# ponimatkin/freepose

Hardware: AMD Instinct MI355X
Metric: proposals/sec (ViT-L feat + top-k + 576-pose render-compare) (higher is better)
Workload: dtype bf16

## Files before the change

freepose_amd/_lib.py:

```python
from __future__ import annotations

import ctypes as C
import os
from pathlib import Path

_HERE = Path(__file__).resolve().parent
LIB_PATH = _HERE / "lib" / "libfreepose_hip.so"
LAB_LIB_PATH = _HERE / "lib" / "libfreepose_hip_lab.so"

_lib = None
_use_lab = False


def use_lab():
    global _use_lab
    if _lib is not None and not _use_lab:
        raise RuntimeError("use_lab() after the product library was loaded")
    _use_lab = True


def is_lab() -> bool:
    return _use_lab

c_void_p, c_int, c_float, c_double, c_size_t, c_char_p = C.c_void_p, C.c_int, C.c_float, C.c_double, C.c_size_t, C.c_char_p
P = C.POINTER


class VitArch(C.Structure):
    _fields_ = [("dim", c_int), ("depth", c_int), ("heads", c_int), ("mlp_dim", c_int), ("patch", c_int),
                ("n_reg", c_int), ("pos_grid", c_int), ("ln_eps", c_float)]


class ClipArch(C.Structure):
    _fields_ = [("width", c_int), ("depth", c_int), ("heads", c_int), ("mlp_dim", c_int), ("patch", c_int), ("grid", c_int),
                ("embed_dim", c_int), ("ln_eps", c_float), ("quick_gelu", c_int)]


class ClipTextArch(C.Structure):
    _fields_ = [("width", c_int), ("depth", c_int), ("heads", c_int), ("mlp_dim", c_int), ("vocab", c_int), ("ctx", c_int),
                ("embed_dim", c_int), ("ln_eps", c_float)]


SIGNATURES = {
    "fp_last_error": (c_char_p, []),
    "fp_version": (c_int, []),
    "fp_ctx_create": (c_int, [c_int, P(c_void_p)]),
    "fp_ctx_destroy": (c_int, [c_void_p]),
    "fp_ctx_set_option": (c_int, [c_void_p, c_char_p, c_int]),
    "fp_ctx_workspace_bytes": (c_size_t, [c_void_p]),
    "fp_vit_create": (c_int, [c_void_p, P(VitArch), P(c_void_p)]),
    "fp_vit_destroy": (c_int, [c_void_p]),
    "fp_vit_set_weight": (c_int, [c_void_p, c_char_p, c_void_p, c_size_t, c_void_p]),
    "fp_vit_forward": (c_int, [c_void_p, c_void_p, c_int, c_int, c_int, c_int, c_int, c_void_p, c_void_p]),
    "fp_vit_flops": (c_double, [c_void_p, c_int, c_int, c_int, c_int]),
    "fp_ffa": (c_int, [c_void_p, c_void_p, c_void_p, c_int, c_int, c_int, c_int, c_int, c_int, c_void_p, c_void_p, c_void_p]),
    "fp_bank_prepare": (c_int, [c_void_p, c_void_p, c_int, c_int, c_void_p, c_void_p]),
    "fp_bank_topk": (c_int, [c_void_p, c_void_p, c_int, c_int, c_void_p, c_int, c_int, c_int, c_void_p, c_void_p, c_void_p]),
    "fp_topk_merge": (c_int, [c_void_p, c_void_p, c_void_p, c_int, c_int, c_int, c_void_p, c_void_p, c_void_p]),
    "fp_rerank_views": (c_int, [c_void_p, c_void_p, c_void_p, c_void_p, c_void_p, c_int, c_int, c_int, c_int, c_void_p, c_void_p]),
    "fp_l2_normalize": (c_int, [c_void_p, c_void_p, c_int, c_int, c_void_p, c_void_p]),
    "fp_template_score": (c_int, [c_void_p, c_void_p, c_void_p, c_void_p, c_int, c_int, c_int, c_void_p, c_void_p]),
    "fp_template_score_normed": (c_int, [c_void_p, c_void_p, c_void_p, c_void_p, c_int, c_int, c_int, c_void_p, c_void_p]),
    "fp_crop_resize_pad": (c_int, [c_void_p, c_void_p, c_int, c_int, c_int, c_int, c_int, c_void_p, c_int, c_float,
                                   c_int, c_void_p, c_int, c_void_p, c_int, c_void_p]),
    "fp_roi_align": (c_int, [c_void_p, c_void_p, c_int, c_int, c_int, c_int, c_void_p, c_int, c_int, c_int, c_int, c_float,
                             c_void_p, c_void_p]),
    "fp_generate_rotations": (c_int, [c_int, c_void_p]),
    "fp_geodesic_select": (c_int, [c_void_p, c_void_p, c_int, c_void_p, c_double, c_void_p, P(c_int), c_void_p]),
    "fp_mesh_upload": (c_int, [c_void_p, c_void_p, c_int, c_void_p, c_int, c_void_p, P(c_void_p)]),
    "fp_mesh_upload_textured": (c_int, [c_void_p, c_void_p, c_int, c_void_p, c_int, c_void_p, c_void_p, c_int, c_int, c_void_p,
                                        P(c_void_p)]),
    "fp_mesh_set_ambient": (c_int, [c_void_p, c_float]),
    "fp_mesh_set_shading": (c_int, [c_void_p, c_int]),
    "fp_mesh_set_filter": (c_int, [c_void_p, c_int]),
    "fp_mesh_set_cull": (c_int, [c_void_p, c_int]),
    "fp_project_vertices": (c_int, [c_void_p, c_void_p, c_void_p, c_int, c_float, c_float, c_float, c_float, c_float, c_void_p,
                                    c_void_p, c_void_p]),
    "fp_mesh_destroy": (c_int, [c_void_p]),
    "fp_rasterize": (c_int, [c_void_p, c_void_p, c_void_p, c_int, c_float, c_float, c_float, c_float, c_float, c_int,
                             c_int, c_void_p, c_void_p, c_void_p]),
    "fp_rasterize_extents": (c_int, [c_void_p, c_void_p, c_void_p, c_int, c_float, c_float, c_float, c_float, c_float, c_int,
                                     c_int, c_void_p, c_void_p, c_void_p, c_void_p, c_void_p]),
    "fp_depth_extents": (c_int, [c_void_p, c_void_p, c_int, c_int, c_int, c_float, c_float, c_float, c_float, c_void_p,
                                 c_void_p]),
    "fp_chamfer": (c_int, [c_void_p, c_void_p, c_int, c_void_p, c_void_p, c_int, c_int, c_int, c_int, c_void_p, c_void_p]),
    "fp_depth_compare": (c_int, [c_void_p, c_void_p, c_void_p, c_int, c_int, c_int, c_void_p, c_int, c_void_p, c_void_p, c_void_p, c_int,
# ... 117 lines not shown
```

freepose_amd/csrc/clip.hip:

```cpp
#include "../../include/freepose_hip.h"
#include "tower_steps.h"

namespace {

constexpr float CLIP_MEAN[3] = {0.48145466f, 0.4578275f, 0.40821073f}, CLIP_SD[3] = {0.26862954f, 0.26130258f, 0.27577711f};

}

struct fp_clip {
    fp_ctx* ctx = nullptr;
    fp_clip_arch a{};
    TowerEmbedW emb;
    const bf16_t *lnprew = nullptr, *lnpreb = nullptr, *lnpostw = nullptr, *lnpostb = nullptr;
    bool have_conv = false;
    ClipTowerCommon tw;
};

extern "C" int fp_clip_create(fp_ctx* ctx, const fp_clip_arch* arch, fp_clip** out) {
    FP_REQUIRE(ctx && arch && out, "clip_create: null argument");
    FP_REQUIRE(arch->quick_gelu == 0, "clip_create: quick_gelu towers are not provided (exact-erf GELU only)");
    if (int rc = ClipTowerCommon::check_arch("clip_create", arch->width, arch->heads, arch->mlp_dim, arch->embed_dim, arch->depth,
                                             arch->patch > 0 && arch->grid > 0, "patch, grid")) return rc;
    fp_clip* v = new fp_clip();
    v->ctx = ctx;
// ... 48 lines not shown
    fp_set_error("clip_set_weight: unknown tensor name '%s'", name);
    return FP_ERR_INVALID;
}

extern "C" int fp_clip_encode_image(fp_clip* v, const void* d_images, int B, int S, void* d_out, void* stream) {
    FP_REQUIRE(v && d_images && d_out, "clip_encode_image: null argument");
    const fp_clip_arch& a = v->a;
    hipStream_t s = (hipStream_t)stream;
    FP_REQUIRE(B > 0, "clip_encode_image: B=%d", B);
    FP_REQUIRE(S == a.patch * a.grid, "clip_encode_image: images are %d x %d, the tower takes %d x %d (patch %d, grid %d: the positional "
               "embedding is not interpolated)", S, S, a.patch * a.grid, a.patch * a.grid, a.patch, a.grid);
    FP_REQUIRE(v->have_conv && v->tw.have_proj && v->emb.cls && v->emb.pos && v->lnprew && v->lnpreb && v->lnpostw && v->lnpostb,
               "clip_encode_image: embedding / ln_pre / ln_post / proj weights not set");
    int rc;
    if ((rc = v->tw.all_blocks_complete("clip_encode_image"))) return rc;
    const int D = a.width, P = a.grid * a.grid, n_tok = P + 1;
    const int npad = cdiv(n_tok, 16) * 16;
    const size_t M = (size_t)B * npad;
    if ((rc = fp_tower_offsets_fit("clip_encode_image", M, D, a.mlp_dim, B))) return rc;

    bf16_t *A0, *X, *Y, *QKV, *AO, *H1, *POOL;
    fp_ctx* ctx = v->ctx;
    FP_WS(ctx, "clip.im2col", (size_t)B * P * v->emb.KP * 2, A0);
    FP_WS(ctx, "clip.x", M * D * 2, X);
    FP_WS(ctx, "clip.y", M * D * 2, Y);
    FP_WS(ctx, "clip.qkv", M * 3 * D * 2, QKV);
    FP_WS(ctx, "clip.ao", M * D * 2, AO);
    FP_WS(ctx, "clip.h1", M * (size_t)a.mlp_dim * 2, H1);
    FP_WS(ctx, "clip.pool", (size_t)B * D * 2, POOL);

    bf16_t* R = Y;
    bf16_t* T = X;
    const TowerRun t{ctx, nullptr, s, B, n_tok, npad, D, a.mlp_dim, a.ln_eps, R, T, AO, H1, v->tw.ones};
    if ((rc = fp_tower_embed(t, v->emb, v->emb.pos + D, (const bf16_t*)d_images, S, S, A0, X))) return rc;
    if ((rc = fp_layernorm(X, Y, v->lnprew, v->lnpreb, (int)M, D, a.ln_eps, 0, 0, 0, s))) return rc;
    if ((rc = fp_tower_blocks(t, v->tw.blk, QKV, a.heads, v->tw.head_dim, false))) return rc;
    if ((rc = fp_layernorm(R, POOL, v->lnpostw, v->lnpostb, B, D, a.ln_eps, 1, npad, 0, s))) return rc;
    return v->tw.project(ctx, POOL, D, a.embed_dim, d_out, B, s);
}

extern "C" double fp_clip_flops(const fp_clip* v, int B) {
    if (!v) return 0.0;
    const fp_clip_arch& a = v->a;
    const double P = (double)a.grid * a.grid, N = P + 1, D = a.width, Mm = a.mlp_dim;
    const double per_block = 8.0 * N * D * D + 4.0 * N * D * Mm + 4.0 * N * N * D;
    return B * (a.depth * per_block + 2.0 * P * (3.0 * a.patch * a.patch) * D + 2.0 * D * a.embed_dim);
}
```

freepose_amd/csrc/tower_steps.h:

```cpp
#pragma once
#include <stdio.h>
#include <string.h>

#include <cmath>

#include "internal.h"

struct GemmStep {
    FpGemmArgs g{};
    int epi;
    GemmStep(const bf16_t* X, int ldx, const bf16_t* W, int K, bf16_t* C, int ldc, const bf16_t* bias, int M, int N, bool gelu = false)
        : epi(gelu ? FP_EPI_BIAS_GELU : FP_EPI_BIAS) {
        g.X = X; g.ldx = ldx; g.W = W; g.ldw = K; g.C = C; g.ldc = ldc; g.bias = bias;
        g.M = M; g.N = N; g.K = K;
    }
    GemmStep& residual(const bf16_t* gamma, const bf16_t* resid, int ldr, float2* stat_part = nullptr) {
        g.gamma = gamma; g.resid = resid; g.ldr = ldr; g.stat_part = stat_part;
        epi = stat_part ? FP_EPI_LS_RES_STATS : FP_EPI_BIAS_LS_RES;
        return *this;
    }
    GemmStep& transposed_v(int npad, int heads) {
        g.ldc = 8; g.npad = npad; g.heads = heads;
        epi = FP_EPI_VT;
        return *this;
// ... 44 lines not shown
            if (hipEventCreate(&e.a) != hipSuccess || hipEventCreate(&e.b) != hipSuccess) return;
            p->ev_pool.push_back(e);
        }
        slot = p->ev_used++;
        p->ev_pool[slot].cls = cls;
        (void)hipEventRecord(p->ev_pool[slot].a, s);
    }
    ~ProfScope() {
        if (slot != (size_t)-1) (void)hipEventRecord(p->ev_pool[slot].b, s);
    }
};

struct TowerBlockW {
    const bf16_t *n1w = nullptr, *n1b = nullptr, *qkvw = nullptr, *qkvb = nullptr, *projw = nullptr,
                 *projb = nullptr, *ls1 = nullptr, *n2w = nullptr, *n2b = nullptr, *fc1w = nullptr, *fc1b = nullptr,
                 *fc2w = nullptr, *fc2b = nullptr, *ls2 = nullptr;
    bool complete() const { return n1w && n1b && qkvw && qkvb && projw && projb && n2w && n2b && fc1w && fc1b && fc2w && fc2b; }
};
struct TowerRun {
    fp_ctx* ctx; TowerProf* prof; hipStream_t s;
    int B, n_tok, npad, D, mlp_dim;
    float eps;
    bf16_t *R, *T, *AO, *H1;
    const bf16_t* ones;
    int M() const { return B * npad; }
    void count(double flops_per_row, int launches) const { if (prof) prof->count((double)B * n_tok * flops_per_row, launches); }
};
struct TowerEmbedW {
    int patch = 0, KP = 0, n_reg = 0;
    const float *mean = nullptr, *sd = nullptr;
    bf16_t* pe_w = nullptr;
    const bf16_t *pe_b = nullptr, *cls = nullptr, *pos = nullptr, *reg = nullptr;
};
inline int fp_tower_embed(const TowerRun& t, const TowerEmbedW& e, const bf16_t* pos_patch, const bf16_t* img, int H, int W, bf16_t* A0, bf16_t* X) {
    const int P = (H / e.patch) * (W / e.patch);
    int rc;
    {
        ProfScope ps(t.prof, t.s, TOWER_OTHER);
        if ((rc = fp_im2col_norm_ms(img, A0, t.B, H, W, e.patch, e.KP, e.mean, e.sd, t.s))) return rc;
        if ((rc = fp_token_init(X, e.cls, e.pos, e.reg, e.n_reg, t.B, t.n_tok, t.npad, t.D, t.s))) return rc;
    }
    ProfScope ps(t.prof, t.s, TOWER_GEMM);
    GemmStep pe(A0, e.KP, e.pe_w, e.KP, X, t.D, e.pe_b, t.B * P, t.D);
    if ((rc = pe.patch_embed(pos_patch, P, t.npad, 1 + e.n_reg).run(t.ctx, t.s))) return rc;
    if (t.prof) t.prof->count(2.0 * t.B * P * (3.0 * e.patch * e.patch) * t.D, 1);
    return FP_OK;
}
inline int fp_tower_out_proj(const TowerRun& t, const TowerBlockW& w, float2* stat_part) {
    ProfScope ps(t.prof, t.s, TOWER_GEMM);
    GemmStep proj(t.AO, t.D, w.projw, t.D, t.R, t.D, w.projb, t.M(), t.D);
    if (int rc = proj.residual(w.ls1 ? w.ls1 : t.ones, t.R, t.D, stat_part).run(t.ctx, t.s)) return rc;
    t.count(2.0 * t.D * t.D, 1);
    return FP_OK;
}
inline int fp_tower_mlp(const TowerRun& t, const TowerBlockW& w, LnStats* st, const bf16_t* fc1w, const uint4* fc1_cb, float2* stat_part) {
    const int D = t.D, M = t.M(), N = t.mlp_dim;
    int rc;
    {
        ProfScope ps(t.prof, t.s, TOWER_OTHER);
        if ((rc = st ? st->ready(nullptr, N, t.s) : fp_layernorm(t.R, t.T, w.n2w, w.n2b, M, D, t.eps, 0, 0, 0, t.s))) return rc;
    }
    ProfScope ps(t.prof, t.s, TOWER_GEMM);
    GemmStep fc1(st ? t.R : t.T, D, st ? fc1w : w.fc1w, D, t.H1, N, w.fc1b, M, N, true);
    if (st && (rc = st->attach(fc1, fc1_cb))) return rc;
    if ((rc = fc1.run(t.ctx, t.s))) return rc;
    if ((rc = GemmStep(t.H1, N, w.fc2w, N, t.R, D, w.fc2b, M, D).residual(w.ls2 ? w.ls2 : t.ones, t.R, D, stat_part).run(t.ctx, t.s))) return rc;
    t.count(4.0 * D * N, 2);
    return FP_OK;
}

inline bool fp_weight_numel(const char* who, const char* name, size_t numel, size_t want) {
    if (numel != want) fp_set_error("%s: %s has %zu elements, expected %zu", who, name, numel, want);
// ... 104 lines not shown
```

freepose_amd/csrc/vit.hip:

```cpp
#include <stdio.h>

#include "../../include/freepose_hip.h"
#include "tower_steps.h"

struct fp_vit {
    fp_ctx* ctx = nullptr;
    fp_vit_arch a{};
    TowerEmbedW emb;
    const bf16_t *normw = nullptr, *normb = nullptr;
    bf16_t* ones = nullptr;
    std::vector<TowerBlockW> blk;
    struct VitFold { bf16_t *qkvw = nullptr, *fc1w = nullptr; uint4 *qkv_cb = nullptr, *fc1_cb = nullptr; };
    std::vector<VitFold> fold;
    int folded_upto = 0;
    hipEvent_t fold_ev = nullptr;
    hipStream_t fold_stream = nullptr;
    bool refold = false;
    std::map<std::pair<int, int>, bf16_t*> pos_cache;
    TowerProf prof;
};

extern "C" int fp_vit_create(fp_ctx* ctx, const fp_vit_arch* arch, fp_vit** out) {
    FP_REQUIRE(ctx && arch && out, "vit_create: null argument");
    FP_REQUIRE(arch->dim % 64 == 0 && arch->heads * 64 == arch->dim, "vit_create: dim=%d heads=%d (head dim must be 64)",
// ... 85 lines not shown
        if (rc) { (void)hipFree(buf); return rc; }
        it = v->pos_cache.emplace(key, buf).first;
    }
    *out = it->second;
    return FP_OK;
}

static int vit_fold(fp_vit* v, int first, int L, hipStream_t s) {
    const fp_vit_arch& a = v->a;
    const size_t D = a.dim, Mm = a.mlp_dim;
    for (int i = first; i < L; ++i) {
        const TowerBlockW& w = v->blk[i];
        fp_vit::VitFold& f = v->fold[i];
        if (!f.qkvw) FP_HIP(hipMalloc((void**)&f.qkvw, 3 * D * D * 2));
        if (!f.qkv_cb) FP_HIP(hipMalloc((void**)&f.qkv_cb, 3 * D * sizeof(uint4)));
        if (!f.fc1w) FP_HIP(hipMalloc((void**)&f.fc1w, Mm * D * 2));
        if (!f.fc1_cb) FP_HIP(hipMalloc((void**)&f.fc1_cb, Mm * sizeof(uint4)));
        int rc;
        if ((rc = fp_ln_fold(w.qkvw, w.n1w, w.n1b, w.qkvb, f.qkvw, f.qkv_cb, (int)(3 * D), (int)D, (int)D, FP_ATTN_QSCALE, s))) return rc;
        if ((rc = fp_ln_fold(w.fc1w, w.n2w, w.n2b, w.fc1b, f.fc1w, f.fc1_cb, (int)Mm, (int)D, 0, 1.0f, s))) return rc;
    }
    return FP_OK;
}

extern "C" double fp_vit_flops(const fp_vit* v, int B, int H, int W, int layer) {
    const fp_vit_arch& a = v->a;
    const double P = (double)(H / a.patch) * (W / a.patch), N = P + 1 + a.n_reg, D = a.dim;
    const int L = std::min(layer, a.depth);
    const double mlp_ratio = (double)a.mlp_dim / a.dim;
    const double per_block = (8.0 + 4.0 * mlp_ratio) * N * D * D + 4.0 * N * N * D;
    return B * (L * per_block + 2.0 * P * (3.0 * a.patch * a.patch) * D);
}

extern "C" int fp_vit_forward(fp_vit* v, const void* d_images, int B, int H, int W, int layer, int feature_type,
                              void* d_out, void* stream) {
    FP_REQUIRE(v && d_images && d_out, "vit_forward: null argument");
    const fp_vit_arch& a = v->a;
    hipStream_t s = (hipStream_t)stream;
    fp_ctx* ctx = v->ctx;
    FP_REQUIRE(B > 0 && H % a.patch == 0 && W % a.patch == 0, "vit_forward: B=%d H=%d W=%d (patch %d)", B, H, W, a.patch);
    FP_REQUIRE(feature_type >= 0 && feature_type <= 3, "vit_forward: feature_type %d", feature_type);
    FP_REQUIRE(v->emb.cls && v->emb.pos && v->emb.pe_b && v->normw && v->normb && (a.n_reg == 0 || v->emb.reg),
               "vit_forward: embedding / final-norm weights not set");
    const int L = (layer >= 1 && layer <= a.depth) ? layer : a.depth;
    for (int i = 0; i < L; ++i) {
        FP_REQUIRE(v->blk[i].complete(), "vit_forward: weights of block %d not set", i);
    }
    const int D = a.dim, gh = H / a.patch, gw = W / a.patch, P = gh * gw;
    const int n_tok = P + 1 + a.n_reg;
    const int npad = cdiv(n_tok, 16) * 16;
    const size_t M = (size_t)B * npad;
    FP_REQUIRE(M * (size_t)a.mlp_dim * 2 < 0xffffffffull, "vit_forward: batch too large for 32-bit tile offsets (B=%d)", B);
    const int Mi = (int)M;

    bf16_t *A0, *X, *Y, *QK, *Vt, *AO, *H1;
    int rc;
    const bool lnf = ctx->opt_ln_fused != 0 && D % 64 == 0;
    LnStats st{nullptr, nullptr, nullptr, Mi, D, a.ln_eps};
    if (lnf) {
        if (v->fold_ev && s != v->fold_stream) FP_HIP(hipStreamWaitEvent(s, v->fold_ev, 0));
        if (v->folded_upto < L) {
            if (v->refold) {
                FP_HIP(hipDeviceSynchronize());
                v->refold = false;
            }
            if ((rc = vit_fold(v, v->folded_upto, L, s))) return rc;
            if (!v->fold_ev) FP_HIP(hipEventCreateWithFlags(&v->fold_ev, hipEventDisableTiming));
            FP_HIP(hipEventRecord(v->fold_ev, s));
            v->fold_stream = s;
            v->folded_upto = L;
        }
        FP_WS(ctx, "vit.ln_stat", M * sizeof(uint4), st.stat);
        FP_WS(ctx, "vit.ln_rstd", M * sizeof(float), st.rstd);
        FP_WS(ctx, "vit.ln_part", M * (size_t)(D / 64) * sizeof(float2), st.part);
    }
    FP_WS(ctx, "vit.im2col", (size_t)B * P * v->emb.KP * 2, A0);
    FP_WS(ctx, "vit.x", M * D * 2, X);
    FP_WS(ctx, "vit.y", M * D * 2, Y);
    FP_WS(ctx, "vit.qk", M * 2 * D * 2, QK);
    FP_WS(ctx, "vit.vt", M * D * 2 + 256, Vt);
    FP_WS(ctx, "vit.ao", M * D * 2, AO);
    FP_WS(ctx, "vit.h1", M * (size_t)a.mlp_dim * 2, H1);

    const bf16_t* pos_patch;
    if ((rc = vit_pos(v, gh, gw, s, &pos_patch))) return rc;

    const TowerRun t{ctx, &v->prof, s, B, n_tok, npad, D, a.mlp_dim, a.ln_eps, X, Y, AO, H1, v->ones};
    if ((rc = fp_tower_embed(t, v->emb, pos_patch, (const bf16_t*)d_images, H, W, A0, X))) return rc;
    const bf16_t* in = lnf ? X : Y;
    for (int i = 0; i < L; ++i) {
        const TowerBlockW& w = v->blk[i];
        const fp_vit::VitFold& f = v->fold[i];
        {
            ProfScope ps(&v->prof, s, TOWER_OTHER);
            if ((rc = lnf ? st.ready(i == 0 ? X : nullptr, 2 * D, s) : fp_layernorm(X, Y, w.n1w, w.n1b, Mi, D, a.ln_eps, 0, 0, 0, s))) return rc;
        }
        {
            ProfScope ps(&v->prof, s, TOWER_GEMM);
            const bf16_t* qkvw = lnf ? f.qkvw : w.qkvw;
            GemmStep qk(in, D, qkvw, D, QK, 2 * D, w.qkvb, Mi, 2 * D), vt(in, D, qkvw + (size_t)2 * D * D, D, Vt, 8, w.qkvb + 2 * D, Mi, D);
            vt.transposed_v(npad, a.heads);
            if (lnf && ((rc = st.attach(qk, f.qkv_cb)) || (rc = st.attach(vt, f.qkv_cb + 2 * D)))) return rc;
            if ((rc = qk.run(ctx, s))) return rc;
            if ((rc = vt.run(ctx, s))) return rc;
            t.count(2.0 * 3.0 * D * D, 2);
        }
        {
            ProfScope ps(&v->prof, s, TOWER_ATTN);
            if ((rc = fp_attention_fwd(QK, 2 * D, Vt, AO, D, B, a.heads, n_tok, npad, lnf, s))) return rc;
        }
        if ((rc = fp_tower_out_proj(t, w, st.part))) return rc;
        if ((rc = fp_tower_mlp(t, w, lnf ? &st : nullptr, f.fc1w, f.fc1_cb, i + 1 < L ? st.part : nullptr))) return rc;
    }
    {
        ProfScope ps(&v->prof, s, TOWER_OTHER);
        const int rows_per_b = feature_type == 0 ? 1 : (feature_type == 1 ? a.n_reg : P);
        const int off = feature_type == 0 ? 0 : (feature_type == 1 ? 1 : 1 + a.n_reg);
        if (rows_per_b > 0)
            if ((rc = fp_layernorm(X, (bf16_t*)d_out, v->normw, v->normb, B * rows_per_b, D, a.ln_eps, rows_per_b, npad,
                                   off, s, feature_type == 3)))
                return rc;
    }
    return FP_OK;
}

extern "C" int fp_vit_profile(fp_vit* v, int enable) {
    FP_REQUIRE(v, "vit_profile: null");
    TowerProf& p = v->prof;
    p.on = enable != 0;
    p.ev_used = 0;
    p.gemm_flops = 0;
    p.gemm_launches = 0;
    return FP_OK;
}
extern "C" int fp_vit_profile_read(fp_vit* v, float* g, float* at, float* o, double* fl) {
    FP_REQUIRE(v, "vit_profile_read: null");
    TowerProf& p = v->prof;
    float acc[3] = {0.f, 0.f, 0.f};
    for (size_t i = 0; i < p.ev_used; ++i) {
        FP_HIP(hipEventSynchronize(p.ev_pool[i].b));
        float ms = 0.f;
        FP_HIP(hipEventElapsedTime(&ms, p.ev_pool[i].a, p.ev_pool[i].b));
        acc[p.ev_pool[i].cls] += ms;
    }
    if (g) *g = acc[TOWER_GEMM];
    if (at) *at = acc[TOWER_ATTN];
    if (o) *o = acc[TOWER_OTHER];
    if (fl) *fl = p.gemm_flops;
    return FP_OK;
}
extern "C" long fp_vit_profile_gemm_launches(const fp_vit* v) { return v ? v->prof.gemm_launches : 0; }
```

freepose_amd/csrc/vit_misc.hip:

```cpp
#include "internal.h"
#include "dot64.h"
#include "gemm_bf16.h"

namespace {

__global__ void im2col_norm_kernel(const bf16_t* __restrict__ img, bf16_t* __restrict__ A, int B, int H,
                                   int W, int ps, int KP, float m0, float m1, float m2, float s0, float s1,
                                   float s2) {
    const int gw = W / ps, gh = H / ps, P = gw * gh;
    const int K = 3 * ps * ps;
    const int chunks = KP / 8;
    const long total = (long)B * P * chunks;
    for (long idx = blockIdx.x * (long)blockDim.x + threadIdx.x; idx < total;
         idx += (long)gridDim.x * blockDim.x) {
        const int ch = (int)(idx % chunks);
        const long row = idx / chunks;
        const int b = (int)(row / P), pp = (int)(row % P);
        const int py = pp / gw, px = pp % gw;
        uint32_t w[4];
#pragma unroll
        for (int e = 0; e < 8; e += 2) {
            float v[2];
#pragma unroll
            for (int u = 0; u < 2; ++u) {
                const int k = ch * 8 + e + u;
                float val = 0.f;
                if (k < K) {
                    const int c = k / (ps * ps), rem = k % (ps * ps);
                    const int dy = rem / ps, dx = rem % ps;
                    const float x = bf2f(img[(((size_t)b * 3 + c) * H + (py * ps + dy)) * W + px * ps + dx]);
                    const float mean = c == 0 ? m0 : (c == 1 ? m1 : m2);
                    const float sd = c == 0 ? s0 : (c == 1 ? s1 : s2);
                    val = rbf(rbf(x - mean) / sd);
                }
                v[u] = val;
            }
            w[e / 2] = pack_bf2(v[0], v[1]);
        }
        *(uint4*)(A + (size_t)row * KP + ch * 8) = make_uint4(w[0], w[1], w[2], w[3]);
    }
}

__global__ void token_init_kernel(bf16_t* __restrict__ X, const bf16_t* __restrict__ cls,
                                  const bf16_t* __restrict__ pos0, const bf16_t* __restrict__ reg, int nreg,
                                  int n_tok, int npad, int D) {
    const int b = blockIdx.y;
    const int nrows = 1 + nreg + (npad - n_tok);
    for (int i = blockIdx.x * blockDim.x + threadIdx.x; i < nrows * D; i += gridDim.x * blockDim.x) {
        const int r = i / D, c = i % D;
        int row;
        bf16_t v;
        if (r == 0) { row = 0; v = f2bf(bf2f(cls[c]) + bf2f(pos0[c])); }
        else if (r <= nreg) { row = r; v = reg[(r - 1) * D + c]; }
        else { row = n_tok + (r - 1 - nreg); v = 0; }
        X[((size_t)b * npad + row) * D + c] = v;
    }
}

template <int MAXC, int L2 = 0>
__global__ __launch_bounds__(256) void layernorm_kernel(const bf16_t* __restrict__ X, bf16_t* __restrict__ Y,
                                                        const bf16_t* __restrict__ gamma,
                                                        const bf16_t* __restrict__ beta, int rows, int D,
                                                        float eps, int rows_per_b, int in_stride_b, int in_off) {
    const int lane = threadIdx.x & 63;
    const int wave = (blockIdx.x * blockDim.x + threadIdx.x) >> 6;
    const int nwave = (gridDim.x * blockDim.x) >> 6;
    const int nch = D / 8;
    for (int r = wave; r < rows; r += nwave) {
        const size_t ir = (size_t)(r / rows_per_b) * in_stride_b + in_off + (r % rows_per_b);
        const bf16_t* xr = X + ir * D;
        uint4 xw[MAXC];
        float v[MAXC][8];
// ... 303 lines not shown

}

int fp_row_stats(const bf16_t* X, uint4* ms, float* rstd, int rows, int D, float eps, hipStream_t s) {
    FP_REQUIRE(D % 8 == 0 && D <= 8 * 64 * 3, "row_stats: D=%d unsupported", D);
    if (rows <= 0) return FP_OK;
    const int blocks = std::min(cdiv(rows, 4), 256 * 8);
    if (D <= 512) hipLaunchKernelGGL(row_stats_kernel<1>, dim3(blocks), dim3(256), 0, s, X, ms, rstd, rows, D, eps);
    else if (D <= 1024) hipLaunchKernelGGL(row_stats_kernel<2>, dim3(blocks), dim3(256), 0, s, X, ms, rstd, rows, D, eps);
    else hipLaunchKernelGGL(row_stats_kernel<3>, dim3(blocks), dim3(256), 0, s, X, ms, rstd, rows, D, eps);
    FP_LAUNCH_CHECK();
    return FP_OK;
}

int fp_stats_finalize(const float2* part, uint4* ms, float* rstd, int rows, int D, float eps, hipStream_t s, int part_ld) {
    FP_REQUIRE(D % 64 == 0, "stats_finalize: D=%d must be a multiple of 64", D);
    if (rows <= 0) return FP_OK;
    hipLaunchKernelGGL(stats_finalize_kernel, dim3(cdiv(rows, 256)), dim3(256), 0, s, part, ms, rstd, rows, D / 64, 1.0f / (float)D, eps, part_ld > 0 ? part_ld : rows);
    FP_LAUNCH_CHECK();
    return FP_OK;
}

int fp_ln_fold(const bf16_t* W, const bf16_t* gamma, const bf16_t* beta, const bf16_t* bias, bf16_t* Wf, uint4* cb, int N, int K,
               int n_scaled, float row_scale, hipStream_t s) {
    FP_REQUIRE(W && gamma && beta && bias && Wf && cb, "ln_fold: null argument (W / LayerNorm gamma, beta / bias / outputs)");
    FP_REQUIRE(N > 0 && K % 8 == 0, "ln_fold: N=%d, K=%d (K must be a multiple of 8)", N, K);
    hipLaunchKernelGGL(ln_fold_kernel, dim3(cdiv(N, 4)), dim3(256), 0, s, W, gamma, beta, bias, Wf, cb, N, K, n_scaled, row_scale);
    FP_LAUNCH_CHECK();
    return FP_OK;
}

int fp_im2col_norm_ms(const bf16_t* img, bf16_t* A, int B, int H, int W, int ps, int KP, const float* mean, const float* sd, hipStream_t s) {
    FP_REQUIRE(H % ps == 0 && W % ps == 0 && KP % 8 == 0 && KP >= 3 * ps * ps, "im2col: bad shape");
    const long total = (long)B * (H / ps) * (W / ps) * (KP / 8);
    const int blocks = (int)std::min<long>((total + 255) / 256, 256 * 16);
    hipLaunchKernelGGL(im2col_norm_kernel, dim3(blocks), dim3(256), 0, s, img, A, B, H, W, ps, KP, rbf(mean[0]), rbf(mean[1]), rbf(mean[2]),
                       rbf(sd[0]), rbf(sd[1]), rbf(sd[2]));
    FP_LAUNCH_CHECK();
    return FP_OK;
}

int fp_token_init(bf16_t* X, const bf16_t* cls, const bf16_t* pos0, const bf16_t* reg, int nreg, int B,
                  int n_tok, int npad, int D, hipStream_t s) {
    const int nrows = 1 + nreg + (npad - n_tok);
    if (B <= 0 || D <= 0) return FP_OK;
    hipLaunchKernelGGL(token_init_kernel, dim3(cdiv(nrows * D, 256), B), dim3(256), 0, s, X, cls, pos0, reg, nreg,
                       n_tok, npad, D);
    FP_LAUNCH_CHECK();
    return FP_OK;
}

int fp_layernorm(const bf16_t* X, bf16_t* Y, const bf16_t* gamma, const bf16_t* beta, int rows, int D, float eps,
                 int rows_per_b, int in_stride_b, int in_off, hipStream_t s, int l2_normalize) {
    FP_REQUIRE(D % 8 == 0 && D <= 8 * 64 * 4, "layernorm: D=%d unsupported", D);
    FP_REQUIRE(!l2_normalize || D <= 8 * 64 * 3, "layernorm: D=%d with l2_normalize unsupported", D);
    if (rows <= 0) return FP_OK;
    if (rows_per_b <= 0) { rows_per_b = rows; in_stride_b = 0; in_off = 0; }
    const int blocks = std::min(cdiv(rows, 4), 256 * 8);
#define FP_LN(C, L) hipLaunchKernelGGL((layernorm_kernel<C, L>), dim3(blocks), dim3(256), 0, s, X, Y, gamma, beta, rows, D, eps, rows_per_b, in_stride_b, in_off)
    if (D <= 512) { if (l2_normalize) FP_LN(1, 1); else FP_LN(1, 0); }
    else if (D <= 1024) { if (l2_normalize) FP_LN(2, 1); else FP_LN(2, 0); }
    else if (D <= 1536) { if (l2_normalize) FP_LN(3, 1); else FP_LN(3, 0); }
    else FP_LN(4, 0);
#undef FP_LN
    FP_LAUNCH_CHECK();
    return FP_OK;
}

int fp_posembed_aa(const bf16_t* src, bf16_t* dst, int G, int gh, int gw, int D, hipStream_t s) {
    FP_REQUIRE(G > 0 && gh > 0 && gw > 0, "posembed: bad grid");
// ... 46 lines not shown
```

freepose_amd/ops.py:

```python
from __future__ import annotations

import ctypes as C
import functools
from typing import Optional

import numpy as np
import torch

from . import _lib
from ._lib import check, current_stream, ptr

_ctx = {}


def context(device: Optional[int] = None):
    if device is None:
        device = torch.cuda.current_device()
    h = _ctx.get(device)
    if h is None:
        lib = _lib.load()
        out = C.c_void_p()
        check(lib.fp_ctx_create(int(device), C.byref(out)), "fp_ctx_create")
        h = _ctx[device] = out
    return h
# ... 33 lines not shown
                 device: Optional[int] = None):
        if model_name not in VIT_ARCHS:
            raise ValueError(f"unknown DINOv2 model {model_name}")
        dim, depth, heads, n_reg = VIT_ARCHS[model_name]
        self.dim, self.depth, self.heads, self.n_reg, self.patch, self.pos_grid = dim, depth, heads, n_reg, 14, 37
        self.lib = _lib.load()
        self.ctx = context(device)
        arch = _lib.VitArch(dim, depth, heads, 4 * dim, 14, n_reg, 37, 1e-6)
        h = C.c_void_p()
        check(self.lib.fp_vit_create(self.ctx, C.byref(arch), C.byref(h)), "fp_vit_create")
        self.handle = h
        self.weights = {}
        if state_dict is None:
            state_dict = random_state_dict(model_name, seed)
        self.load_state_dict(state_dict)

    def load_state_dict(self, sd: dict):
        s = current_stream()
        for name, t in sd.items():
            if name == "mask_token":
                continue
            w = _dev(torch.as_tensor(t), torch.bfloat16)
            self.weights[name] = w
            check(self.lib.fp_vit_set_weight(self.handle, name.encode(), ptr(w), w.numel(), s), f"set_weight({name})")
        torch.cuda.synchronize()

    def forward(self, images: torch.Tensor, layer: int = 22, feature_type: str = "cls",
                out: Optional[torch.Tensor] = None) -> torch.Tensor:
        x = _dev(images, torch.bfloat16)
        B, Cc, H, W = x.shape
        assert Cc == 3
        P = (H // self.patch) * (W // self.patch)
        ft = FEATURE_TYPES[feature_type]
        shape = {0: (B, self.dim), 1: (B, self.n_reg, self.dim), 2: (B, P, self.dim), 3: (B, P, self.dim)}[ft]
        if out is None:
            out = torch.empty(shape, dtype=torch.bfloat16, device=x.device)
        else:
            assert tuple(out.shape) == shape and out.dtype == torch.bfloat16 and out.is_contiguous() and out.device == x.device
        if B > 0:
            check(self.lib.fp_vit_forward(self.handle, ptr(x), B, H, W, int(layer), ft, ptr(out), current_stream()),
                  "fp_vit_forward")
        return out

    __call__ = forward

    def flops(self, B, H, W, layer=22) -> float:
        return float(self.lib.fp_vit_flops(self.handle, B, H, W, layer))

    def profile(self, enable: bool):
        check(self.lib.fp_vit_profile(self.handle, int(enable)))

    def profile_read(self):
        g, a, o, f = C.c_float(), C.c_float(), C.c_float(), C.c_double()
        check(self.lib.fp_vit_profile_read(self.handle, C.byref(g), C.byref(a), C.byref(o), C.byref(f)))
        return {"ms_gemm": g.value, "ms_attn": a.value, "ms_other": o.value, "gemm_flops": f.value,
                "gemm_launches": int(self.lib.fp_vit_profile_gemm_launches(self.handle))}

    def __del__(self):
        try:
            self.lib.fp_vit_destroy(self.handle)
        except Exception:
            pass


def random_state_dict(model_name: str, seed: int = 0) -> dict:
    dim, depth, heads, n_reg = VIT_ARCHS[model_name]
    g = torch.Generator().manual_seed(seed)

    def tn(*shape, std=0.02):
        return torch.nn.init.trunc_normal_(torch.empty(*shape), std=std, a=-2 * std, b=2 * std, generator=g)

    sd = {"cls_token": tn(1, 1, dim, std=1e-6) + 0.0, "pos_embed": tn(1, 1 + 37 * 37, dim),
          "patch_embed.proj.weight": tn(dim, 3, 14, 14), "patch_embed.proj.bias": tn(dim),
          "norm.weight": torch.ones(dim), "norm.bias": torch.zeros(dim)}
    sd["cls_token"] = tn(1, 1, dim)
    if n_reg:
        sd["register_tokens"] = tn(1, n_reg, dim)
# ... 1300 lines not shown
```

freepose_amd/pipeline.py:

```python
from __future__ import annotations

from dataclasses import dataclass
from typing import List, Optional

import numpy as np
import torch

from freepose_amd import ops, parallel
from freepose_amd.retrieval import TemplateBank
from freepose_amd.src.pipeline.retrieval.renderer import MeshRenderer, grid_poses
from freepose_amd.src.pipeline.utils import z_from_extents


class StageClock:

    def __init__(self):
        self._spans = []
        self._pool = []

    class _Span:
        def __init__(self, clock, name):
            self.clock, self.name = clock, name

        def __enter__(self):
# ... 50 lines not shown
        self.fx = self.fy = 600.0 * render_res / 420.0
        self.cx = self.cy = render_res / 2
        self.clock = _NoClock()

    def retrieve(self, crops: torch.Tensor, masks: torch.Tensor):
        with self.clock.stage("vit_query"):
            feats = self.vit(crops, layer=self.layer, feature_type="patch")
        g = self.crop_res // 14
        with self.clock.stage("ffa"):
            desc = ops.ffa(feats, masks[:, : g * 14, : g * 14], cell=14, normalize=True)
        with self.clock.stage("bank_scan_topk"):
            s, i = self.bank.topk(desc, self.k)
        return feats, s, i

    def render_hypotheses(self):
        with self.clock.stage("rasterize"):
            rgb, _, ext, boxes = ops.rasterize_extents(self.mesh, self._poses_dev, self.render_scale, self.fx, self.fy, self.cx, self.cy,
                                                       self.render_res, self.render_res)
        with self.clock.stage("crop_resize"):
            crops = ops.crop_resize_pad(rgb, boxes, self.crop_res, 0.0, out_bf16=True)
        return crops, ext

    def hypothesis_features(self, crops: torch.Tensor, normalized: bool = False) -> torch.Tensor:
        g = self.crop_res // 14
        sizes = ops.plan_vit_batches(crops.shape[0], g * g + 5, self.vit_batch)
        with self.clock.stage("vit_hypotheses"):
            feats = torch.empty((crops.shape[0], g * g, self.vit.dim), dtype=torch.bfloat16, device=crops.device)
            i = 0
            for b in sizes:
                self.vit(crops[i:i + b], layer=self.layer, feature_type="patch_normalized" if normalized else "patch", out=feats[i:i + b])
                i += b
            return feats

    def run(self, crops: torch.Tensor, masks: torch.Tensor, K: np.ndarray, bboxes: np.ndarray, scales) -> List[ProposalResult]:
        feats, top_s, top_i = self.retrieve(crops, masks)
        out = []
        for b in range(crops.shape[0]):
            hyp_crops, ext = self.render_hypotheses()
            hyp_feats = self.hypothesis_features(hyp_crops, normalized=True)
            with self.clock.stage("template_score"):
                q = ops.l2_normalize(feats[b])
                scores = ops.template_score(hyp_feats, q, normalized=True)
            with self.clock.stage("hypothesis_top3"):
                idx_all = torch.arange(self.n_hyp, dtype=torch.int32, device=scores.device)
                s3, i3 = ops.topk_merge(scores[None], idx_all[None], 3)
            k = top_s.shape[1]
            packed = torch.cat([i3[0].double(), s3[0].double(), ext[i3[0].long(), 4:6].double().reshape(-1), top_s[b].double(),
                                top_i[b].double()]).cpu().numpy()
            i3h = packed[0:3].astype(np.int64)
            s3h = packed[3:6].astype(np.float32)
            e = packed[6:12].reshape(3, 2)
            ratio = float(scales[b]) / self.render_scale
            tco = [z_from_extents(bboxes[b], e[j, 0] * ratio, e[j, 1] * ratio, K, self.hyp_poses[i3h[j]]) for j in range(3)]
            out.append(ProposalResult(packed[12:12 + k].astype(np.float32), packed[12 + k:12 + 2 * k].astype(np.int32), i3h, s3h, tco))
        return out


def pack_results(results: List[ProposalResult]) -> torch.Tensor:
    rows = [[float(r.topk_idx[0]), float(r.topk_scores[0]), float(r.hyp_idx[0]), float(r.hyp_scores[0]),
             *r.TCO[0][:3, :3].flatten().tolist(), *r.TCO[0][:3, 3].tolist()] for r in results]
    return torch.tensor(rows, dtype=torch.float64).reshape(-1, 16)
```

include/freepose_hip.h:

```cpp
#ifndef FREEPOSE_HIP_H
#define FREEPOSE_HIP_H
#include <stddef.h>
#include <stdint.h>

#ifdef __cplusplus
extern "C" {
#endif

#define FP_OK 0
#define FP_ERR_INVALID 1
#define FP_ERR_HIP 2
#define FP_ERR_STATE 3

typedef struct fp_ctx fp_ctx;
typedef struct fp_vit fp_vit;
typedef struct fp_mesh fp_mesh;

const char* fp_last_error(void);
int fp_version(void);
int fp_ctx_create(int device, fp_ctx** out);
int fp_ctx_destroy(fp_ctx* ctx);
int fp_ctx_set_option(fp_ctx* ctx, const char* name, int value);
size_t fp_ctx_workspace_bytes(const fp_ctx* ctx);

typedef struct {
    int dim;
    int depth;
    int heads;
    int mlp_dim;
    int patch;
    int n_reg;
    int pos_grid;
    float ln_eps;
} fp_vit_arch;

int fp_vit_create(fp_ctx* ctx, const fp_vit_arch* arch, fp_vit** out);
int fp_vit_destroy(fp_vit* vit);
int fp_vit_set_weight(fp_vit* vit, const char* name, const void* d_bf16, size_t numel, void* stream);
int fp_vit_forward(fp_vit* vit, const void* d_images, int B, int H, int W, int layer, int feature_type,
                   void* d_out_bf16, void* stream);
double fp_vit_flops(const fp_vit* vit, int B, int H, int W, int layer);

int fp_ffa(fp_ctx* ctx, const void* d_feats, const uint8_t* d_mask, int B, int gh, int gw, int D, int cell,
           int normalize, void* d_out_bf16, float* d_out_f32, void* stream);

int fp_bank_prepare(fp_ctx* ctx, const float* d_bank_f32, int N, int D, void* d_bank_bf16, void* stream);
int fp_bank_topk(fp_ctx* ctx, const void* d_bank_bf16, int N, int D, const void* d_queries, int Q, int k,
                 int idx_offset, float* d_out_scores, int32_t* d_out_idx, void* stream);
int fp_topk_merge(fp_ctx* ctx, const float* d_cand_scores, const int32_t* d_cand_idx, int Q, int C, int k,
                  float* d_out_scores, int32_t* d_out_idx, void* stream);
int fp_rerank_views(fp_ctx* ctx, const void* d_views, const int32_t* d_offsets, const int32_t* d_cand,
                    const void* d_queries, int Q, int C, int D, int k, float* d_out, void* stream);
int fp_l2_normalize(fp_ctx* ctx, const void* d_x_bf16, int rows, int D, void* d_y_bf16, void* stream);

int fp_template_score(fp_ctx* ctx, const void* d_tmpl, const void* d_query, const float* d_weights, int T, int P,
                      int D, float* d_scores, void* stream);
int fp_template_score_normed(fp_ctx* ctx, const void* d_tmpl_normed, const void* d_query, const float* d_weights, int T,
                             int P, int D, float* d_scores, void* stream);

int fp_crop_resize_pad(fp_ctx* ctx, const void* d_images, int src_fmt, int n_img, int C, int H, int W,
                       const int32_t* d_boxes, int n, float bbox_extend, int target, const uint8_t* d_masks,
                       int mask_mode, void* d_out, int out_fmt, void* stream);

int fp_roi_align(fp_ctx* ctx, const float* d_images, int n_img, int C, int H, int W, const float* d_rois, int n,
                 int pooled_h, int pooled_w, int sampling_ratio, float spatial_scale, float* d_out, void* stream);

int fp_generate_rotations(int n, double* h_out);
int fp_geodesic_select(fp_ctx* ctx, const double* d_grid, int G, const double* h_Rprev9, double thresh_deg,
                       int32_t* d_out_idx, int* h_n, void* stream);

int fp_mesh_upload(fp_ctx* ctx, const float* h_verts, int V, const int32_t* h_faces, int F,
                   const uint8_t* h_colors, fp_mesh** out);
int fp_mesh_upload_textured(fp_ctx* ctx, const float* h_verts, int V, const int32_t* h_faces, int F, const float* h_uv,
// ... 150 lines not shown
```

Before: 1.999.

## Batch query crop with hypothesis crops in one multi-part ViT forward

Adds a multi-part ViT forward that runs several image groups, each with its own output feature type, through one batched tower pass. The pipeline now puts each query crop into the first hypothesis ViT batch instead of running a separate retrieval ViT pass, and runs FFA and bank top-k per proposal. It also adds a row-wise LDS-staged im2col kernel with vectorised loads to replace the scattered per-element im2col. The aim is fewer small ViT launches and better batch fill, at the cost of per-proposal FFA and top-k calls.

```diff
diff --git a/freepose_amd/_lib.py b/freepose_amd/_lib.py
--- a/freepose_amd/_lib.py
+++ b/freepose_amd/_lib.py
@@ -52,6 +52,7 @@
     "fp_vit_destroy": (c_int, [c_void_p]),
     "fp_vit_set_weight": (c_int, [c_void_p, c_char_p, c_void_p, c_size_t, c_void_p]),
     "fp_vit_forward": (c_int, [c_void_p, c_void_p, c_int, c_int, c_int, c_int, c_int, c_void_p, c_void_p]),
+    "fp_vit_forward_parts": (c_int, [c_void_p, c_int, P(c_void_p), P(c_int), P(c_int), P(c_void_p), c_int, c_int, c_int, c_void_p]),
     "fp_vit_flops": (c_double, [c_void_p, c_int, c_int, c_int, c_int]),
     "fp_ffa": (c_int, [c_void_p, c_void_p, c_void_p, c_int, c_int, c_int, c_int, c_int, c_int, c_void_p, c_void_p, c_void_p]),
     "fp_bank_prepare": (c_int, [c_void_p, c_void_p, c_int, c_int, c_void_p, c_void_p]),
diff --git a/freepose_amd/csrc/clip.hip b/freepose_amd/csrc/clip.hip
--- a/freepose_amd/csrc/clip.hip
+++ b/freepose_amd/csrc/clip.hip
@@ -104,7 +104,8 @@
     bf16_t* R = Y;
     bf16_t* T = X;
     const TowerRun t{ctx, nullptr, s, B, n_tok, npad, D, a.mlp_dim, a.ln_eps, R, T, AO, H1, v->tw.ones};
-    if ((rc = fp_tower_embed(t, v->emb, v->emb.pos + D, (const bf16_t*)d_images, S, S, A0, X))) return rc;
+    const bf16_t* images = (const bf16_t*)d_images;
+    if ((rc = fp_tower_embed(t, v->emb, v->emb.pos + D, TowerImages(&images, &B), S, S, A0, X))) return rc;
     if ((rc = fp_layernorm(X, Y, v->lnprew, v->lnpreb, (int)M, D, a.ln_eps, 0, 0, 0, s))) return rc;
     if ((rc = fp_tower_blocks(t, v->tw.blk, QKV, a.heads, v->tw.head_dim, false))) return rc;
     if ((rc = fp_layernorm(R, POOL, v->lnpostw, v->lnpostb, B, D, a.ln_eps, 1, npad, 0, s))) return rc;
diff --git a/freepose_amd/csrc/tower_steps.h b/freepose_amd/csrc/tower_steps.h
--- a/freepose_amd/csrc/tower_steps.h
+++ b/freepose_amd/csrc/tower_steps.h
@@ -100,12 +100,19 @@
     bf16_t* pe_w = nullptr;
     const bf16_t *pe_b = nullptr, *cls = nullptr, *pos = nullptr, *reg = nullptr;
 };
-inline int fp_tower_embed(const TowerRun& t, const TowerEmbedW& e, const bf16_t* pos_patch, const bf16_t* img, int H, int W, bf16_t* A0, bf16_t* X) {
+struct TowerImages {
+    int n_parts; const bf16_t* const* img; const int* count;
+    TowerImages(int n, const bf16_t* const* im, const int* cnt) : n_parts(n), img(im), count(cnt) {}
+    TowerImages(const bf16_t* const* one, const int* B) : n_parts(1), img(one), count(B) {}
+};
+inline int fp_tower_embed(const TowerRun& t, const TowerEmbedW& e, const bf16_t* pos_patch, const TowerImages& im, int H, int W, bf16_t* A0, bf16_t* X) {
     const int P = (H / e.patch) * (W / e.patch);
     int rc;
     {
         ProfScope ps(t.prof, t.s, TOWER_OTHER);
-        if ((rc = fp_im2col_norm_ms(img, A0, t.B, H, W, e.patch, e.KP, e.mean, e.sd, t.s))) return rc;
+        size_t crop0 = 0;
+        for (int i = 0; i < im.n_parts; crop0 += im.count[i++])
+            if ((rc = fp_im2col_norm_ms(im.img[i], A0 + crop0 * P * e.KP, im.count[i], H, W, e.patch, e.KP, e.mean, e.sd, t.s))) return rc;
         if ((rc = fp_token_init(X, e.cls, e.pos, e.reg, e.n_reg, t.B, t.n_tok, t.npad, t.D, t.s))) return rc;
     }
     ProfScope ps(t.prof, t.s, TOWER_GEMM);
diff --git a/freepose_amd/csrc/vit.hip b/freepose_amd/csrc/vit.hip
--- a/freepose_amd/csrc/vit.hip
+++ b/freepose_amd/csrc/vit.hip
@@ -141,25 +141,33 @@
     return B * (L * per_block + 2.0 * P * (3.0 * a.patch * a.patch) * D);
 }
 
-extern "C" int fp_vit_forward(fp_vit* v, const void* d_images, int B, int H, int W, int layer, int feature_type,
-                              void* d_out, void* stream) {
-    FP_REQUIRE(v && d_images && d_out, "vit_forward: null argument");
+static int vit_forward_parts(const char* who, fp_vit* v, int n_parts, const void* const* d_images, const int* counts, const int* feature_types,
+                             void* const* d_outs, int H, int W, int layer, void* stream) {
+    FP_REQUIRE(v && n_parts > 0 && d_images && counts && feature_types && d_outs, "%s: null argument", who);
     const fp_vit_arch& a = v->a;
     hipStream_t s = (hipStream_t)stream;
     fp_ctx* ctx = v->ctx;
-    FP_REQUIRE(B > 0 && H % a.patch == 0 && W % a.patch == 0, "vit_forward: B=%d H=%d W=%d (patch %d)", B, H, W, a.patch);
-    FP_REQUIRE(feature_type >= 0 && feature_type <= 3, "vit_forward: feature_type %d", feature_type);
+    long Bl = 0;
+    for (int i = 0; i < n_parts; ++i) {
+        FP_REQUIRE(counts[i] >= 0, "%s: part %d has %d crops", who, i, counts[i]);
+        if (counts[i] == 0) continue;
+        FP_REQUIRE(d_images[i] && d_outs[i], "%s: null argument (images / output of part %d)", who, i);
+        FP_REQUIRE(feature_types[i] >= 0 && feature_types[i] <= 3, "%s: feature_type %d", who, feature_types[i]);
+        Bl += counts[i];
+    }
+    FP_REQUIRE(Bl > 0 && Bl <= 0x7fffffffl && H % a.patch == 0 && W % a.patch == 0, "%s: B=%ld H=%d W=%d (patch %d)", who, Bl, H, W, a.patch);
+    const int B = (int)Bl;
     FP_REQUIRE(v->emb.cls && v->emb.pos && v->emb.pe_b && v->normw && v->normb && (a.n_reg == 0 || v->emb.reg),
-               "vit_forward: embedding / final-norm weights not set");
+               "%s: embedding / final-norm weights not set", who);
     const int L = (layer >= 1 && layer <= a.depth) ? layer : a.depth;
     for (int i = 0; i < L; ++i) {
-        FP_REQUIRE(v->blk[i].complete(), "vit_forward: weights of block %d not set", i);
+        FP_REQUIRE(v->blk[i].complete(), "%s: weights of block %d not set", who, i);
     }
     const int D = a.dim, gh = H / a.patch, gw = W / a.patch, P = gh * gw;
     const int n_tok = P + 1 + a.n_reg;
     const int npad = cdiv(n_tok, 16) * 16;
     const size_t M = (size_t)B * npad;
-    FP_REQUIRE(M * (size_t)a.mlp_dim * 2 < 0xffffffffull, "vit_forward: batch too large for 32-bit tile offsets (B=%d)", B);
+    FP_REQUIRE(M * (size_t)a.mlp_dim * 2 < 0xffffffffull, "%s: batch too large for 32-bit tile offsets (B=%d)", who, B);
     const int Mi = (int)M;
 
     bf16_t *A0, *X, *Y, *QK, *Vt, *AO, *H1;
@@ -195,7 +203,7 @@
     if ((rc = vit_pos(v, gh, gw, s, &pos_patch))) return rc;
 
     const TowerRun t{ctx, &v->prof, s, B, n_tok, npad, D, a.mlp_dim, a.ln_eps, X, Y, AO, H1, v->ones};
-    if ((rc = fp_tower_embed(t, v->emb, pos_patch, (const bf16_t*)d_images, H, W, A0, X))) return rc;
+    if ((rc = fp_tower_embed(t, v->emb, pos_patch, TowerImages(n_parts, (const bf16_t* const*)d_images, counts), H, W, A0, X))) return rc;
     const bf16_t* in = lnf ? X : Y;
     for (int i = 0; i < L; ++i) {
         const TowerBlockW& w = v->blk[i];
@@ -223,14 +231,29 @@
     }
     {
         ProfScope ps(&v->prof, s, TOWER_OTHER);
-        const int rows_per_b = feature_type == 0 ? 1 : (feature_type == 1 ? a.n_reg : P);
-        const int off = feature_type == 0 ? 0 : (feature_type == 1 ? 1 : 1 + a.n_reg);
-        if (rows_per_b > 0)
-            if ((rc = fp_layernorm(X, (bf16_t*)d_out, v->normw, v->normb, B * rows_per_b, D, a.ln_eps, rows_per_b, npad,
-                                   off, s, feature_type == 3)))
-                return rc;
-    }
-    return FP_OK;
+        size_t crop0 = 0;
+        for (int i = 0; i < n_parts; crop0 += counts[i++]) {
+            const int ft = feature_types[i];
+            const int rows_per_b = ft == 0 ? 1 : (ft == 1 ? a.n_reg : P);
+            const int off = ft == 0 ? 0 : (ft == 1 ? 1 : 1 + a.n_reg);
+            if (counts[i] > 0 && rows_per_b > 0)
+                if ((rc = fp_layernorm(X + crop0 * npad * D, (bf16_t*)d_outs[i], v->normw, v->normb, counts[i] * rows_per_b, D, a.ln_eps,
+                                       rows_per_b, npad, off, s, ft == 3)))
+                    return rc;
+        }
+    }
+    return FP_OK;
+}
+
+extern "C" int fp_vit_forward(fp_vit* v, const void* d_images, int B, int H, int W, int layer, int feature_type,
+                              void* d_out, void* stream) {
+    FP_REQUIRE(v && d_images && d_out, "vit_forward: null argument");
+    FP_REQUIRE(B > 0, "vit_forward: B=%d H=%d W=%d (patch %d)", B, H, W, v->a.patch);
+    return vit_forward_parts("vit_forward", v, 1, &d_images, &B, &feature_type, &d_out, H, W, layer, stream);
+}
+extern "C" int fp_vit_forward_parts(fp_vit* v, int n_parts, const void* const* d_images, const int* counts, const int* feature_types,
+                                    void* const* d_outs, int H, int W, int layer, void* stream) {
+    return vit_forward_parts("vit_forward_parts", v, n_parts, d_images, counts, feature_types, d_outs, H, W, layer, stream);
 }
 
 extern "C" int fp_vit_profile(fp_vit* v, int enable) {
diff --git a/freepose_amd/csrc/vit_misc.hip b/freepose_amd/csrc/vit_misc.hip
--- a/freepose_amd/csrc/vit_misc.hip
+++ b/freepose_amd/csrc/vit_misc.hip
@@ -38,6 +38,94 @@
             w[e / 2] = pack_bf2(v[0], v[1]);
         }
         *(uint4*)(A + (size_t)row * KP + ch * 8) = make_uint4(w[0], w[1], w[2], w[3]);
+    }
+}
+
+constexpr int IM2COL_THREADS = 512;
+constexpr int IM2COL_PAD = 16;
+constexpr int IM2COL_MAX_LDS = 64 * 1024;
+constexpr int IM2COL_MAX_INDEX = 1 << 22;
+
+__device__ __forceinline__ void divmod_small(int i, int d, float rcp, int& q, int& r) {
+    q = (int)((float)i * rcp);
+    r = i - q * d;
+    if (r < 0) { --q; r += d; }
+    else if (r >= d) { ++q; r -= d; }
+}
+
+template <int V> struct Im2colLoad;
+template <> struct Im2colLoad<1> { typedef uint16_t type; };
+template <> struct Im2colLoad<2> { typedef uint32_t type; };
+template <> struct Im2colLoad<4> { typedef uint2 type; };
+template <> struct Im2colLoad<8> { typedef uint4 type; };
+
+template <int V>
+__global__ __launch_bounds__(IM2COL_THREADS) void im2col_norm_rows_kernel(const bf16_t* __restrict__ img, bf16_t* __restrict__ A, int H,
+                                                                          int W, int ps, int gw, int KP, float rcp_w, float rcp_ps,
+                                                                          float m0, float m1, float m2, float s0, float s1, float s2) {
+    extern __shared__ uint4 im2col_lds[];
+    bf16_t* T = (bf16_t*)im2col_lds;
+    typedef typename Im2colLoad<V>::type load_t;
+    constexpr int UNR = 4;
+    const int py = blockIdx.x, gh = gridDim.x, b = blockIdx.y;
+    const int pp = ps * ps, K = 3 * pp, LP = KP + IM2COL_PAD;
+    const int lane = threadIdx.x & 63, wave = threadIdx.x >> 6;
+    for (int px = wave; px < gw; px += IM2COL_THREADS / 64)
+        for (int k = K + lane; k < KP; k += 64) T[px * LP + k] = 0;
+    const int nchunk = ps * W / V;
+    for (int c = 0; c < 3; ++c) {
+        const load_t* src = (const load_t*)(img + (((size_t)b * 3 + c) * H + (size_t)py * ps) * W);
+        const float mean = c == 0 ? m0 : (c == 1 ? m1 : m2);
+        const float sd = c == 0 ? s0 : (c == 1 ? s1 : s2);
+        for (int j0 = threadIdx.x; j0 < nchunk; j0 += UNR * IM2COL_THREADS) {
+            load_t raw[UNR];
+#pragma unroll
+            for (int u = 0; u < UNR; ++u) {
+                const int j = j0 + u * IM2COL_THREADS;
+                if (j < nchunk) raw[u] = src[j];
+            }
+#pragma unroll
+            for (int u = 0; u < UNR; ++u) {
+                const int j = j0 + u * IM2COL_THREADS;
+                if (j >= nchunk) break;
+                uint16_t x[V];
+                __builtin_memcpy(x, &raw[u], sizeof(load_t));
+                int dy, col, px, dx;
+                divmod_small(j * V, W, rcp_w, dy, col);
+                divmod_small(col, ps, rcp_ps, px, dx);
+                int o = px * LP + c * pp + dy * ps + dx;
+                constexpr int E = V == 1 ? 1 : 2;
+#pragma unroll
+                for (int e = 0; e < V; e += E) {
+                    const float v0 = rbf(bf2f(x[e]) - mean) / sd;
+                    if constexpr (V == 1) {
+                        T[o] = f2bf(v0);
+                    } else {
+                        const float v1 = rbf(bf2f(x[e + 1]) - mean) / sd;
+                        *(uint32_t*)(T + o) = pack_bf2(v0, v1);
+                    }
+                    dx += E;
+                    o += E;
+                    if (dx == ps) {
+                        dx = 0;
+                        o += LP - ps;
+                        if (++px == gw) {
+                            px = 0;
+                            o += ps - gw * LP;
+                        }
+                    }
+                }
+            }
+        }
+    }
+    __syncthreads();
+    const int chunks = KP / 8, nout = gw * chunks;
+    const float rcp_chunks = 1.0f / (float)chunks;
+    uint4* dst = (uint4*)(A + ((size_t)b * gh + py) * gw * (size_t)KP);
+    for (int i = threadIdx.x; i < nout; i += IM2COL_THREADS) {
+        int px, ch;
+        divmod_small(i, chunks, rcp_chunks, px, ch);
+        dst[i] = *(const uint4*)(T + px * LP + ch * 8);
     }
 }
 
@@ -407,10 +495,28 @@
 
 int fp_im2col_norm_ms(const bf16_t* img, bf16_t* A, int B, int H, int W, int ps, int KP, const float* mean, const float* sd, hipStream_t s) {
     FP_REQUIRE(H % ps == 0 && W % ps == 0 && KP % 8 == 0 && KP >= 3 * ps * ps, "im2col: bad shape");
-    const long total = (long)B * (H / ps) * (W / ps) * (KP / 8);
-    const int blocks = (int)std::min<long>((total + 255) / 256, 256 * 16);
-    hipLaunchKernelGGL(im2col_norm_kernel, dim3(blocks), dim3(256), 0, s, img, A, B, H, W, ps, KP, rbf(mean[0]), rbf(mean[1]), rbf(mean[2]),
-                       rbf(sd[0]), rbf(sd[1]), rbf(sd[2]));
+    if (B <= 0) return FP_OK;
+    const float m0 = rbf(mean[0]), m1 = rbf(mean[1]), m2 = rbf(mean[2]), s0 = rbf(sd[0]), s1 = rbf(sd[1]), s2 = rbf(sd[2]);
+    const int gh = H / ps, gw = W / ps;
+    const size_t lds = (size_t)gw * (KP + IM2COL_PAD) * 2;
+    const bool fits = lds <= (size_t)IM2COL_MAX_LDS && (long)ps * W < IM2COL_MAX_INDEX && (long)gw * (KP / 8) < IM2COL_MAX_INDEX && B <= 65535 &&
+                      ((uintptr_t)A & 15) == 0;
+    if (!fits) {
+        const long total = (long)B * gh * gw * (KP / 8);
+        const int blocks = (int)std::min<long>((total + 255) / 256, 256 * 16);
+        hipLaunchKernelGGL(im2col_norm_kernel, dim3(blocks), dim3(256), 0, s, img, A, B, H, W, ps, KP, m0, m1, m2, s0, s1, s2);
+        FP_LAUNCH_CHECK();
+        return FP_OK;
+    }
+    const uintptr_t align = (uintptr_t)img | ((uintptr_t)H * W * 2) | ((uintptr_t)ps * W * 2);
+    const int V = ps % 2 ? 1 : (align % 16 == 0 ? 8 : (align % 8 == 0 ? 4 : (align % 4 == 0 ? 2 : 1)));
+#define FP_IM2COL(VV) hipLaunchKernelGGL(im2col_norm_rows_kernel<VV>, dim3(gh, B), dim3(IM2COL_THREADS), lds, s, img, A, H, W, ps, gw, KP, \
+                                         1.0f / (float)W, 1.0f / (float)ps, m0, m1, m2, s0, s1, s2)
+    if (V == 8) FP_IM2COL(8);
+    else if (V == 4) FP_IM2COL(4);
+    else if (V == 2) FP_IM2COL(2);
+    else FP_IM2COL(1);
+#undef FP_IM2COL
     FP_LAUNCH_CHECK();
     return FP_OK;
 }
diff --git a/freepose_amd/ops.py b/freepose_amd/ops.py
--- a/freepose_amd/ops.py
+++ b/freepose_amd/ops.py
@@ -89,7 +89,7 @@
         assert Cc == 3
         P = (H // self.patch) * (W // self.patch)
         ft = FEATURE_TYPES[feature_type]
-        shape = {0: (B, self.dim), 1: (B, self.n_reg, self.dim), 2: (B, P, self.dim), 3: (B, P, self.dim)}[ft]
+        shape = self._out_shape(B, P, ft)
         if out is None:
             out = torch.empty(shape, dtype=torch.bfloat16, device=x.device)
         else:
@@ -100,6 +100,30 @@
         return out
 
     __call__ = forward
+
+    def _out_shape(self, B: int, P: int, ft: int) -> tuple:
+        return {0: (B, self.dim), 1: (B, self.n_reg, self.dim), 2: (B, P, self.dim), 3: (B, P, self.dim)}[ft]
+
+    def forward_parts(self, parts, layer: int = 22) -> list:
+        xs, fts, outs = [], [], []
+        for images, feature_type, out in parts:
+            x = _dev(images, torch.bfloat16)
+            assert x.dim() == 4 and x.shape[1] == 3 and (not xs or x.shape[2:] == xs[0].shape[2:]), "parts must share 3 x H x W"
+            ft = FEATURE_TYPES[feature_type]
+            shape = self._out_shape(x.shape[0], (x.shape[2] // self.patch) * (x.shape[3] // self.patch), ft)
+            if out is None:
+                out = torch.empty(shape, dtype=torch.bfloat16, device=x.device)
+            else:
+                assert tuple(out.shape) == shape and out.dtype == torch.bfloat16 and out.is_contiguous() and out.device == x.device
+            xs.append(x), fts.append(ft), outs.append(out)
+        n = len(xs)
+        if sum(x.shape[0] for x in xs) > 0:
+            H, W = xs[0].shape[2:]
+            check(self.lib.fp_vit_forward_parts(self.handle, n, (C.c_void_p * n)(*[x.data_ptr() for x in xs]),
+                                                (C.c_int * n)(*[x.shape[0] for x in xs]), (C.c_int * n)(*fts),
+                                                (C.c_void_p * n)(*[o.data_ptr() for o in outs]), int(H), int(W), int(layer),
+                                                current_stream()), "fp_vit_forward_parts")
+        return outs
 
     def flops(self, B, H, W, layer=22) -> float:
         return float(self.lib.fp_vit_flops(self.handle, B, H, W, layer))
diff --git a/freepose_amd/pipeline.py b/freepose_amd/pipeline.py
--- a/freepose_amd/pipeline.py
+++ b/freepose_amd/pipeline.py
@@ -106,21 +106,37 @@
                 i += b
             return feats
 
+    def _query_and_hypothesis_features(self, query: torch.Tensor, crops: torch.Tensor):
+        g = self.crop_res // 14
+        sizes = ops.plan_vit_batches(crops.shape[0] + 1, g * g + 5, self.vit_batch)
+        with self.clock.stage("vit_hypotheses"):
+            feats = torch.empty((crops.shape[0], g * g, self.vit.dim), dtype=torch.bfloat16, device=crops.device)
+            i = sizes[0] - 1
+            qfeat, _ = self.vit.forward_parts([(query, "patch", None), (crops[:i], "patch_normalized", feats[:i])], layer=self.layer)
+            for b in sizes[1:]:
+                self.vit(crops[i:i + b], layer=self.layer, feature_type="patch_normalized", out=feats[i:i + b])
+                i += b
+        return qfeat, feats
+
     def run(self, crops: torch.Tensor, masks: torch.Tensor, K: np.ndarray, bboxes: np.ndarray, scales) -> List[ProposalResult]:
-        feats, top_s, top_i = self.retrieve(crops, masks)
+        g = self.crop_res // 14
         out = []
         for b in range(crops.shape[0]):
             hyp_crops, ext = self.render_hypotheses()
-            hyp_feats = self.hypothesis_features(hyp_crops, normalized=True)
+            feats, hyp_feats = self._query_and_hypothesis_features(crops[b:b + 1], hyp_crops)
+            with self.clock.stage("ffa"):
+                desc = ops.ffa(feats, masks[b:b + 1, : g * 14, : g * 14], cell=14, normalize=True)
+            with self.clock.stage("bank_scan_topk"):
+                top_s, top_i = self.bank.topk(desc, self.k)
             with self.clock.stage("template_score"):
-                q = ops.l2_normalize(feats[b])
+                q = ops.l2_normalize(feats[0])
                 scores = ops.template_score(hyp_feats, q, normalized=True)
             with self.clock.stage("hypothesis_top3"):
                 idx_all = torch.arange(self.n_hyp, dtype=torch.int32, device=scores.device)
                 s3, i3 = ops.topk_merge(scores[None], idx_all[None], 3)
             k = top_s.shape[1]
-            packed = torch.cat([i3[0].double(), s3[0].double(), ext[i3[0].long(), 4:6].double().reshape(-1), top_s[b].double(),
-                                top_i[b].double()]).cpu().numpy()
+            packed = torch.cat([i3[0].double(), s3[0].double(), ext[i3[0].long(), 4:6].double().reshape(-1), top_s[0].double(),
+                                top_i[0].double()]).cpu().numpy()
             i3h = packed[0:3].astype(np.int64)
             s3h = packed[3:6].astype(np.float32)
             e = packed[6:12].reshape(3, 2)
diff --git a/include/freepose_hip.h b/include/freepose_hip.h
--- a/include/freepose_hip.h
+++ b/include/freepose_hip.h
@@ -39,6 +39,8 @@
 int fp_vit_set_weight(fp_vit* vit, const char* name, const void* d_bf16, size_t numel, void* stream);
 int fp_vit_forward(fp_vit* vit, const void* d_images, int B, int H, int W, int layer, int feature_type,
                    void* d_out_bf16, void* stream);
+int fp_vit_forward_parts(fp_vit* vit, int n_parts, const void* const* d_images, const int* counts, const int* feature_types,
+                         void* const* d_outs_bf16, int H, int W, int layer, void* stream);
 double fp_vit_flops(const fp_vit* vit, int B, int H, int W, int layer);
 
 int fp_ffa(fp_ctx* ctx, const void* d_feats, const uint8_t* d_mask, int B, int gh, int gw, int D, int cell,
```

New measurement: 2.016, median of 6. Within noise of the previous version (+0.9%).
